# ducha-aiki/affnet

Measured on NVIDIA H100. Metric: Mpix/s end-to-end HesAffNet(+OriNet)+HardNet, higher is better.
Workload: dtype fp16 operands (fp16 residual planes: AffNet/OriNet weights+activations, HardNet layer 2-3 weights), fp32 accumulate; stencils fp32

## Files before the change

affnet_b200/csrc/pyramid.cu:

```cuda
#include <math.h>
#include <stdarg.h>

#include <string>
#include <vector>

#include <cuda.h>

#include "common.cuh"
#include "pyramid_fused.cuh"

namespace ag {

static thread_local char g_err[512] = "";
thread_local int g_launches = 0;

void set_error(const char* fmt, ...) {
    va_list ap;
    va_start(ap, fmt);
    vsnprintf(g_err, sizeof(g_err), fmt, ap);
    va_end(ap);
}

struct Prof {
    bool on = false;
    cudaStream_t st = nullptr;
    std::vector<cudaEvent_t> ev;
    std::vector<std::string> names;
    std::vector<float> ms;
};
static Prof g_prof;

void prof_mark(const char* name) {
    if (!g_prof.on) return;
    cudaEvent_t e;
    if (cudaEventCreate(&e) != cudaSuccess) return;
    cudaEventRecord(e, g_prof.st);
    g_prof.ev.push_back(e);
    g_prof.names.push_back(name);
}

constexpr int kMaxRadius = 12;
struct BlurTaps {
    int r;
    float w[2 * kMaxRadius + 1];
};

int gauss_kernel_size(double sigma) {
    int k = (int)(2.0 * 3.0 * sigma + 1.0);
    if (k % 2 == 0) k += 1;
    return k;
}

int make_taps(double sigma, BlurTaps* t) {
    int k = gauss_kernel_size(sigma);
    if (k < 1 || k > 2 * kMaxRadius + 1) {
        set_error("gaussian sigma %.4f needs %d taps (max %d)", sigma, k, 2 * kMaxRadius + 1);
        return AG_ERR_INVALID;
    }
    double half = k / 2.0, e[2 * kMaxRadius + 1], sum = 0.0;
    double step = (k > 1) ? (2.0 * half) / (k - 1) : 0.0;
    for (int i = 0; i < k; i++) {
        double x = (i == k - 1) ? half : -half + i * step;
        e[i] = exp(-(x * x) / (2.0 * sigma * sigma));
        sum += e[i];
    }
    t->r = k / 2;
    for (int i = 0; i < k; i++) t->w[i] = (float)(e[i] / sum);
    return AG_OK;
}

constexpr int TW = 64, TH = 64, NT = 256;

template <int R>
struct BlurGeom {
    static constexpr int IH = TH + 2 * R;
    static constexpr int IWQ = (TW + 2 * R + 3) / 4 + 1;
    static constexpr int IW = IWQ * 4;
    static constexpr int NQ = (4 + 2 * R + 3) / 4 + 1;
    static constexpr size_t SMEM = sizeof(float) * ((size_t)IH * IW + (size_t)IH * TW);
};

template <int R>
__global__ void __launch_bounds__(NT) blur_kernel(const float* __restrict__ in, float* __restrict__ out,
                                                   float* __restrict__ dec, int h, int w, BlurTaps taps,
                                                   const __grid_constant__ CUtensorMap tmap, int use_tmap) {
    using G = BlurGeom<R>;
    extern __shared__ __align__(128) float smem_f[];
    float* s_in = smem_f;
    float* s_mid = smem_f + G::IH * G::IW;
    constexpr int R4 = (R + 3) / 4 * 4;
    const int b = blockIdx.z;
    const int x0 = blockIdx.x * TW, y0 = blockIdx.y * TH;
    const float* img = in + (size_t)b * h * w;
#ifndef AG_BLUR_SCALAR_FILL
    const bool wide = (w & 3) == 0 && x0 - R4 >= 0 && x0 - R4 + G::IW <= w && (reinterpret_cast<size_t>(img) & 15) == 0;
#ifndef AG_BLUR_LDG_FILL
    __shared__ __align__(8) unsigned long long s_bar;
    const bool bulk = wide && y0 - R >= 0 && y0 - R + G::IH <= h;
    if (bulk) {
        const uint32_t bar = (uint32_t)__cvta_generic_to_shared(&s_bar);
        if (threadIdx.x == 0) {
            asm volatile("mbarrier.init.shared::cta.b64 [%0], 1;" ::"r"(bar));
            asm volatile("fence.mbarrier_init.release.cluster;" ::: "memory");
            asm volatile("mbarrier.arrive.expect_tx.shared::cta.b64 _, [%0], %1;" ::"r"(bar), "r"((uint32_t)(G::IH * G::IW * 4)) : "memory");
        }
        __syncthreads();
        if (use_tmap) {
            if (threadIdx.x == 0)
                asm volatile("cp.async.bulk.tensor.3d.shared::cluster.global.tile.mbarrier::complete_tx::bytes [%0], [%1, {%2, %3, %4}], [%5];" ::"r"(
                                 (uint32_t)__cvta_generic_to_shared(s_in)),
                             "l"(reinterpret_cast<uint64_t>(&tmap)), "r"(x0 - R4), "r"(y0 - R), "r"(b), "r"(bar)
                             : "memory");
        } else if ((threadIdx.x & 31) == 0) {
            const float* src = img + (size_t)(y0 - R) * w + (x0 - R4);
            for (int ly = threadIdx.x >> 5; ly < G::IH; ly += NT / 32)
                asm volatile("cp.async.bulk.shared::cluster.global.mbarrier::complete_tx::bytes [%0], [%1], %2, [%3];" ::"r"(
                                 (uint32_t)__cvta_generic_to_shared(s_in + ly * G::IW)),
                             "l"(src + (size_t)ly * w), "r"((uint32_t)(G::IW * 4)), "r"(bar)
                             : "memory");
        }
        if (threadIdx.x < 32)
            asm volatile("{\n .reg .pred P;\n W_%=:\n mbarrier.try_wait.parity.shared::cta.b64 P, [%0], 0;\n @P bra D_%=;\n bra W_%=;\n D_%=:\n}\n" ::"r"(bar) : "memory");
    } else
#endif
    if (wide) {
        constexpr int QW = G::IW / 4;
        static_assert(G::IW % 4 == 0, "window rows are whole float4s");
        for (int i = threadIdx.x; i < G::IH * QW; i += NT) {
            const int ly = i / QW, q = i - ly * QW;
            const int gy = clampi(y0 + ly - R, 0, h - 1);
            reinterpret_cast<float4*>(s_in)[i] = __ldg(reinterpret_cast<const float4*>(img + (size_t)gy * w + (x0 - R4)) + q);
        }
    } else
#endif
    for (int i = threadIdx.x; i < G::IH * G::IW; i += NT) {
        const int ly = i / G::IW, lx = i - ly * G::IW;
        const int gy = clampi(y0 + ly - R, 0, h - 1), gx = clampi(x0 + lx - R4, 0, w - 1);
        s_in[i] = __ldg(img + (size_t)gy * w + gx);
    }
    __syncthreads();
    for (int i = threadIdx.x; i < G::IH * (TW / 4); i += NT) {
        const int ly = i / (TW / 4), q = i - ly * (TW / 4);
        constexpr int OFF = R4 - R;
        float v[G::NQ * 4];
        const float4* row = reinterpret_cast<const float4*>(s_in + ly * G::IW + q * 4);
#pragma unroll
        for (int j = 0; j < G::NQ; j++) {
            const float4 t = row[j];
            v[4 * j] = t.x; v[4 * j + 1] = t.y; v[4 * j + 2] = t.z; v[4 * j + 3] = t.w;
        }
        float4 o = make_float4(0.f, 0.f, 0.f, 0.f);
#pragma unroll
        for (int k = 0; k <= 2 * R; k++) {
            const float wk = taps.w[k];
            o.x = fmaf(wk, v[OFF + k], o.x); o.y = fmaf(wk, v[OFF + k + 1], o.y);
            o.z = fmaf(wk, v[OFF + k + 2], o.z); o.w = fmaf(wk, v[OFF + k + 3], o.w);
        }
        *reinterpret_cast<float4*>(s_mid + ly * TW + q * 4) = o;
    }
    __syncthreads();
    const int h2 = (h + 1) >> 1, w2 = (w + 1) >> 1;
    const bool vec_ok = (w & 3) == 0 && (reinterpret_cast<size_t>(out) & 15) == 0;
    {
        const int q = threadIdx.x & 15, rb = threadIdx.x >> 4;
        float4 acc[4];
#pragma unroll
        for (int r = 0; r < 4; r++) acc[r] = make_float4(0.f, 0.f, 0.f, 0.f);
#pragma unroll
        for (int k = 0; k < 4 + 2 * R; k++) {
            const float4 t = *reinterpret_cast<const float4*>(s_mid + (rb * 4 + k) * TW + q * 4);
#pragma unroll
            for (int r = 0; r < 4; r++) {
                const int tap = k - r;
                if (tap >= 0 && tap <= 2 * R) {
                    const float wk = taps.w[tap];
                    acc[r].x = fmaf(wk, t.x, acc[r].x); acc[r].y = fmaf(wk, t.y, acc[r].y);
                    acc[r].z = fmaf(wk, t.z, acc[r].z); acc[r].w = fmaf(wk, t.w, acc[r].w);
                }
            }
        }
        const int gx = x0 + q * 4;
#pragma unroll
        for (int r = 0; r < 4; r++) {
            const int gy = y0 + rb * 4 + r;
            if (gy >= h || gx >= w) continue;
            float* orow = out + (size_t)b * h * w + (size_t)gy * w + gx;
            const float vals[4] = {acc[r].x, acc[r].y, acc[r].z, acc[r].w};
            if (vec_ok) {
                *reinterpret_cast<float4*>(orow) = acc[r];
            } else {
#pragma unroll
                for (int e = 0; e < 4; e++)
                    if (gx + e < w) orow[e] = vals[e];
            }
            if (dec != nullptr && (gy & 1) == 0) {
                float* drow = dec + (size_t)b * h2 * w2 + (size_t)(gy >> 1) * w2 + (gx >> 1);
                drow[0] = vals[0];
                if (gx + 2 < w) drow[1] = vals[2];
            }
        }
    }
}

typedef CUresult (*TmapEncodeFn)(CUtensorMap*, CUtensorMapDataType, cuuint32_t, void*, const cuuint64_t*, const cuuint64_t*, const cuuint32_t*,
                                 const cuuint32_t*, CUtensorMapInterleave, CUtensorMapSwizzle, CUtensorMapL2promotion, CUtensorMapFloatOOBfill);
static TmapEncodeFn tmap_encoder() {
    static TmapEncodeFn fn = nullptr;
    static bool tried = false;
    if (!tried) {
        tried = true;
        if (getenv("AG_BLUR_NO_TMA") == nullptr) {
            void* p = nullptr;
            cudaDriverEntryPointQueryResult q;
            if (cudaGetDriverEntryPoint("cuTensorMapEncodeTiled", &p, cudaEnableDefault, &q) == cudaSuccess && q == cudaDriverEntryPointSuccess)
                fn = reinterpret_cast<TmapEncodeFn>(p);
            else
                cudaGetLastError();
        }
    }
    return fn;
}

static bool make_level_tmap(CUtensorMap* m, const float* base, int B, int h, int w, int iw, int ih) {
    TmapEncodeFn enc = tmap_encoder();
    if (enc == nullptr || (w & 3) != 0 || (reinterpret_cast<size_t>(base) & 15) != 0 || iw > 256 || ih > 256) return false;
    const cuuint64_t dims[3] = {(cuuint64_t)w, (cuuint64_t)h, (cuuint64_t)B};
    const cuuint64_t strides[2] = {(cuuint64_t)w * 4, (cuuint64_t)w * h * 4};
    const cuuint32_t box[3] = {(cuuint32_t)iw, (cuuint32_t)ih, 1};
    const cuuint32_t estr[3] = {1, 1, 1};
    return enc(m, CU_TENSOR_MAP_DATA_TYPE_FLOAT32, 3, const_cast<float*>(base), dims, strides, box, estr, CU_TENSOR_MAP_INTERLEAVE_NONE,
               CU_TENSOR_MAP_SWIZZLE_NONE, CU_TENSOR_MAP_L2_PROMOTION_NONE, CU_TENSOR_MAP_FLOAT_OOB_FILL_NONE) == CUDA_SUCCESS;
}

static int launch_blur(const float* in, float* out, float* dec, int B, int h, int w, double sigma, cudaStream_t st) {
    BlurTaps taps;
    int rc = make_taps(sigma, &taps);
    if (rc != AG_OK) return rc;
    dim3 grid(cdiv(w, TW), cdiv(h, TH), B), block(NT);
    CUtensorMap tmap;
    memset(&tmap, 0, sizeof(tmap));
    switch (taps.r) {
#define AG_BLUR_CASE(R)                                                                                                   \
    case R: {                                                                                                             \
        static SmemAttrOnce attr_once;                                                                                    \
        rc = attr_once.ensure(blur_kernel<R>, BlurGeom<R>::SMEM, "blur smem attr");                                       \
        if (rc != AG_OK) return rc;                                                                                       \
        const int use_tmap = make_level_tmap(&tmap, in, B, h, w, BlurGeom<R>::IW, BlurGeom<R>::IH) ? 1 : 0;                 \
        blur_kernel<R><<<grid, block, BlurGeom<R>::SMEM, st>>>(in, out, dec, h, w, taps, tmap, use_tmap);                  \
    } break;
        AG_BLUR_CASE(1) AG_BLUR_CASE(2) AG_BLUR_CASE(3) AG_BLUR_CASE(4) AG_BLUR_CASE(5) AG_BLUR_CASE(6)
        AG_BLUR_CASE(7) AG_BLUR_CASE(8) AG_BLUR_CASE(9) AG_BLUR_CASE(10) AG_BLUR_CASE(11) AG_BLUR_CASE(12)
#undef AG_BLUR_CASE
        default:
            set_error("unsupported blur radius %d", taps.r);
            return AG_ERR_INVALID;
    }
    AG_CHECK_LAUNCH("blur_kernel");
    return AG_OK;
}

static int g_pyr_fused = 0;

static int num_sms_pyr() {
    static int n = 0;
    if (n == 0) {
        int dev = 0;
        cudaGetDevice(&dev);
        cudaDeviceGetAttribute(&n, cudaDevAttrMultiProcessorCount, dev);
        if (n <= 0) n = 148;
    }
    return n;
}

template <int CH>
static int launch_octave(const float* src, float* const* outs, float* dec, int seed, int B, int h, int w, const double* sigmas, cudaStream_t st, bool* handled) {
    using C = pf::Chain<CH>;
    *handled = false;
    if ((w & 3) != 0 || w < 8 || h < 2) return AG_OK;
    if ((reinterpret_cast<size_t>(src) & 15) || (dec && (reinterpret_cast<size_t>(dec) & 15))) return AG_OK;
    for (int l = 0; l < C::NB; l++)
        if (reinterpret_cast<size_t>(outs[l]) & 15) return AG_OK;
    pf::OctArgs a;
    memset(&a, 0, sizeof(a));
    for (int l = 0; l < C::NB; l++) {
        BlurTaps t;
        int rc = make_taps(sigmas[l], &t);
        if (rc != AG_OK) return rc;
        if (t.r != C::R(l)) return AG_OK;
        for (int k = 0; k <= 2 * t.r; k++) a.taps[l][k] = t.w[k];
        a.out[l] = outs[l];
    }
    a.src = src; a.dec = dec; a.seed = seed; a.B = B; a.h = h; a.w = w;
    a.nstrips = cdiv(w, pf::SWMAX);
    a.sw = cdiv(cdiv(w, a.nstrips), 4) * 4;
    a.nstrips = cdiv(w, a.sw);
    int nb = (2 * num_sms_pyr() + a.nstrips * B - 1) / (a.nstrips * B);
    const int nb_max = h / 48 > 1 ? h / 48 : 1;
    if (nb > nb_max) nb = nb_max;
    if (nb < 1) nb = 1;
    a.band = cdiv(h, nb);
    a.nbands = cdiv(h, a.band);
    static bool configured[64] = {};
    int dev = 0;
    cudaGetDevice(&dev);
    if (!configured[dev & 63]) {
        int rc = check_cuda(cudaFuncSetAttribute(pf::octave_kernel<CH>, cudaFuncAttributeMaxDynamicSharedMemorySize, (int)sizeof(pf::Smem<CH>)), "octave smem attr");
        if (rc != AG_OK) return rc;
        configured[dev & 63] = true;
    }
    pf::octave_kernel<CH><<<dim3(a.nstrips * a.nbands, B), 64 * C::NB, sizeof(pf::Smem<CH>), st>>>(a);
    AG_CHECK_LAUNCH("octave_kernel");
    *handled = true;
    return AG_OK;
}

__global__ void decimate_kernel(const float* __restrict__ in, float* __restrict__ out, int h, int w, int h2, int w2) {
    int x = blockIdx.x * blockDim.x + threadIdx.x, y = blockIdx.y, b = blockIdx.z;
    if (x < w2) out[(size_t)b * h2 * w2 + (size_t)y * w2 + x] = in[(size_t)b * h * w + (size_t)(2 * y) * w + 2 * x];
}

}

using namespace ag;

extern "C" {

const char* ag_last_error(void) { return ag::g_err; }
int ag_abi_version(void) { return 1; }

int ag_prof_begin(void* stream) {
    for (cudaEvent_t e : g_prof.ev) cudaEventDestroy(e);
    g_prof.ev.clear(); g_prof.names.clear(); g_prof.ms.clear();
    g_prof.st = (cudaStream_t)stream;
    g_prof.on = true;
    prof_mark("<begin>");
    return AG_OK;
}

int ag_prof_end(void) {
    g_prof.on = false;
    if (g_prof.ev.empty()) return 0;
    int rc = check_cuda(cudaEventSynchronize(g_prof.ev.back()), "prof sync");
    if (rc != AG_OK) return rc;
    g_prof.ms.assign(g_prof.ev.size(), 0.f);
    for (size_t i = 1; i < g_prof.ev.size(); i++) cudaEventElapsedTime(&g_prof.ms[i], g_prof.ev[i - 1], g_prof.ev[i]);
    return (int)g_prof.ev.size() - 1;
}

int ag_prof_get(int i, const char** name, float* ms) {
    AG_REQUIRE(i >= 0 && (size_t)(i + 1) < g_prof.ev.size() && name && ms, "index out of range");
    *name = g_prof.names[i + 1].c_str();
    *ms = g_prof.ms[i + 1];
    return AG_OK;
}

int ag_pyramid_plan(int B, int H, int W, int nlevels, double init_sigma, int border, ag_pyramid_plan_t* plan) {
    AG_REQUIRE(plan != nullptr, "plan is NULL");
    AG_REQUIRE(B >= 1 && H >= 1 && W >= 1, "bad image size");
    AG_REQUIRE(nlevels >= 1 && nlevels + 2 <= AG_MAX_LEVELS, "nlevels out of range");
    memset(plan, 0, sizeof(*plan));
    plan->B = B; plan->H = H; plan->W = W;
    plan->n_levels = nlevels + 2;
    const double sigma_step = pow(2.0, 1.0 / (double)nlevels);
    const int min_size = 2 * border + 2 + 1;
    double cur_sigma = 0.5, first = 0.0, pd = 1.0;
    if (init_sigma > cur_sigma) {
        first = sqrt(init_sigma * init_sigma - cur_sigma * cur_sigma);
        cur_sigma = init_sigma;
    }
    int h = H, w = W, o = 0;
    long long off = 0;
    for (;;) {
        AG_REQUIRE(o < AG_MAX_OCTAVES, "too many octaves");
        plan->h[o] = h; plan->w[o] = w; plan->pix_dist[o] = pd;
        plan->sigma[o][0] = cur_sigma;
        plan->blur_sigma[o][0] = (o == 0) ? first : 0.0;
        for (int l = 0; l < plan->n_levels; l++) {
            plan->level_offset[o][l] = off;
            off += (long long)B * h * w;
        }
        for (int i = 1; i < plan->n_levels; i++) {
            plan->blur_sigma[o][i] = cur_sigma * sqrt(sigma_step * sigma_step - 1.0);
            cur_sigma = cur_sigma * sigma_step;
            plan->sigma[o][i] = cur_sigma;
        }
        o++;
        pd *= 2.0;
        cur_sigma = init_sigma;
        int nh = (h + 1) / 2, nw = (w + 1) / 2;
        if (nh <= min_size || nw <= min_size) break;
        h = nh; w = nw;
    }
    plan->n_octaves = o;
    plan->total_floats = off;
    return AG_OK;
}

int ag_debug_pyramid_mode(int fused) {
    const int old = g_pyr_fused;
    g_pyr_fused = fused ? 1 : 0;
    return old;
}

int ag_gaussian_blur(const float* d_in, float* d_out, int B, int h, int w, double sigma, void* stream) {
    AG_REQUIRE(d_in && d_out && B >= 1 && h >= 1 && w >= 1, "bad arguments");
    return launch_blur(d_in, d_out, nullptr, B, h, w, sigma, (cudaStream_t)stream);
}

int ag_pyramid_build(const ag_pyramid_plan_t* p, const float* d_img, float* d_pyr, void* stream) {
    AG_REQUIRE(p && d_img && d_pyr, "NULL argument");
    cudaStream_t st = (cudaStream_t)stream;
    const int nl = p->n_levels, seed_level = nl - 2;
    for (int o = 0; o < p->n_octaves; o++)
        for (int l = (o == 0 && p->blur_sigma[0][0] > 0.0) ? 0 : 1; l < nl; l++) {
            BlurTaps t;
            int rc = make_taps(p->blur_sigma[o][l], &t);
            if (rc != AG_OK) return rc;
        }
    static const bool env_fused = getenv("AG_PYR_FUSED") != nullptr;
    const bool no_fused = !(env_fused || g_pyr_fused);
    for (int o = 0; o < p->n_octaves; o++) {
        const int h = p->h[o], w = p->w[o];
        float* lvl0 = d_pyr + p->level_offset[o][0];
        float* next0 = (o + 1 < p->n_octaves) ? d_pyr + p->level_offset[o + 1][0] : nullptr;
        if (nl == 5 && !no_fused) {
            bool handled = false;
            int rc;
            if (o == 0 && p->blur_sigma[0][0] > 0.0) {
                float* outs[5];
                double sg[5];
                for (int l = 0; l < 5; l++) { outs[l] = d_pyr + p->level_offset[0][l]; sg[l] = p->blur_sigma[0][l]; }
                rc = launch_octave<0>(d_img, outs, next0, seed_level, p->B, h, w, sg, st, &handled);
            } else if (o > 0) {
                float* outs[4];
                double sg[4];
                for (int l = 1; l < 5; l++) { outs[l - 1] = d_pyr + p->level_offset[o][l]; sg[l - 1] = p->blur_sigma[o][l]; }
                rc = launch_octave<1>(lvl0, outs, next0, seed_level - 1, p->B, h, w, sg, st, &handled);
            } else rc = AG_OK;
            if (rc != AG_OK) return rc;
            if (handled) continue;
        }
        if (o == 0) {
            if (p->blur_sigma[0][0] > 0.0) {
                int rc = launch_blur(d_img, lvl0, nullptr, p->B, h, w, p->blur_sigma[0][0], st);
                if (rc != AG_OK) return rc;
            } else {
                int rc = check_cuda(cudaMemcpyAsync(lvl0, d_img, sizeof(float) * (size_t)p->B * h * w,
                                                    cudaMemcpyDeviceToDevice, st), "copy level 0");
                if (rc != AG_OK) return rc;
            }
        }
        for (int l = 1; l < nl; l++) {
            float* dec = (l == seed_level && o + 1 < p->n_octaves) ? d_pyr + p->level_offset[o + 1][0] : nullptr;
            int rc = launch_blur(d_pyr + p->level_offset[o][l - 1], d_pyr + p->level_offset[o][l], dec, p->B, h, w,
                                 p->blur_sigma[o][l], st);
            if (rc != AG_OK) return rc;
        }
    }
    return AG_OK;
}

}
```

Baseline: 670.7.

## Fuse small-octave pyramid tail into one shared-memory kernel per image

From octave 3 onward, once the octave fits in shared memory, all remaining blur levels and decimations are built by a single per-image kernel that keeps working planes in shared memory. This removes the many small per-level blur launches whose fixed overhead dominates at small resolutions. The tail is handled with only B blocks, so it uses few SMs and could be slow if B is small. It also requires identical taps across the tail octaves and falls back to the old path otherwise.

```diff
diff --git a/affnet_b200/csrc/pyramid.cu b/affnet_b200/csrc/pyramid.cu
--- a/affnet_b200/csrc/pyramid.cu
+++ b/affnet_b200/csrc/pyramid.cu
@@ -202,6 +202,107 @@
     }
 }
 
+constexpr int TAIL_NT = 1024;
+
+struct TailArgs {
+    const float* seed;
+    float* lvl[AG_MAX_OCTAVES][AG_MAX_LEVELS];
+    int h[AG_MAX_OCTAVES], w[AG_MAX_OCTAVES];
+    int r[AG_MAX_LEVELS];
+    float taps[AG_MAX_LEVELS][2 * kMaxRadius + 1];
+    int n_oct, nl, seed_level;
+};
+
+template <int R>
+__device__ __forceinline__ void tail_hpass(const float* __restrict__ a, float* __restrict__ m, int h, int w, const float* __restrict__ wt) {
+    const int nq = (w + 3) >> 2;
+    for (int i = threadIdx.x; i < h * nq; i += TAIL_NT) {
+        const int y = i / nq, x0 = (i - y * nq) * 4;
+        const float* row = a + y * w;
+        float v[4 + 2 * R];
+#pragma unroll
+        for (int j = 0; j < 4 + 2 * R; j++) v[j] = row[clampi(x0 - R + j, 0, w - 1)];
+        float o[4] = {0.f, 0.f, 0.f, 0.f};
+#pragma unroll
+        for (int k = 0; k <= 2 * R; k++) {
+            const float wk = wt[k];
+#pragma unroll
+            for (int e = 0; e < 4; e++) o[e] = fmaf(wk, v[k + e], o[e]);
+        }
+#pragma unroll
+        for (int e = 0; e < 4; e++)
+            if (x0 + e < w) m[y * w + x0 + e] = o[e];
+    }
+}
+
+template <int R>
+__device__ __forceinline__ void tail_vpass(const float* __restrict__ m, float* __restrict__ a, float* __restrict__ g, float* __restrict__ d,
+                                           float* __restrict__ gd, int h, int w, const float* __restrict__ wt) {
+    const int nr = (h + 3) >> 2, w2 = (w + 1) >> 1;
+    for (int i = threadIdx.x; i < nr * w; i += TAIL_NT) {
+        const int yq = i / w, x = i - yq * w, y0 = yq * 4;
+        float v[4 + 2 * R];
+#pragma unroll
+        for (int j = 0; j < 4 + 2 * R; j++) v[j] = m[clampi(y0 - R + j, 0, h - 1) * w + x];
+        float o[4] = {0.f, 0.f, 0.f, 0.f};
+#pragma unroll
+        for (int k = 0; k <= 2 * R; k++) {
+            const float wk = wt[k];
+#pragma unroll
+            for (int e = 0; e < 4; e++) o[e] = fmaf(wk, v[k + e], o[e]);
+        }
+#pragma unroll
+        for (int e = 0; e < 4; e++) {
+            const int y = y0 + e;
+            if (y >= h) break;
+            a[y * w + x] = o[e];
+            g[y * w + x] = o[e];
+            if (d != nullptr && ((y | x) & 1) == 0) {
+                d[(y >> 1) * w2 + (x >> 1)] = o[e];
+                if (gd != nullptr) gd[(y >> 1) * w2 + (x >> 1)] = o[e];
+            }
+        }
+    }
+}
+
+__global__ void __launch_bounds__(TAIL_NT) pyramid_tail_kernel(const __grid_constant__ TailArgs p) {
+    extern __shared__ __align__(16) float tail_smem[];
+    const int b = blockIdx.x;
+    const int h0 = p.h[0], w0 = p.w[0];
+    float* a = tail_smem;
+    float* m = a + h0 * w0;
+    float* d = m + h0 * w0;
+    {
+        const float* src = p.seed + (size_t)b * h0 * w0;
+        for (int i = threadIdx.x; i < h0 * w0; i += TAIL_NT) a[i] = src[i];
+    }
+    for (int o = 0; o < p.n_oct; o++) {
+        const int h = p.h[o], w = p.w[o];
+        if (o > 0)
+            for (int i = threadIdx.x; i < h * w; i += TAIL_NT) a[i] = d[i];
+        __syncthreads();
+        for (int l = 1; l < p.nl; l++) {
+            const float* wt = p.taps[l];
+            float* g = p.lvl[o][l] + (size_t)b * h * w;
+            const bool seed = l == p.seed_level && o + 1 < p.n_oct;
+            float* gd = seed ? p.lvl[o + 1][0] + (size_t)b * p.h[o + 1] * p.w[o + 1] : nullptr;
+            switch (p.r[l]) {
+#define AG_TAIL_CASE(RR)                                                             \
+    case RR:                                                                         \
+        tail_hpass<RR>(a, m, h, w, wt);                                              \
+        __syncthreads();                                                             \
+        tail_vpass<RR>(m, a, g, seed ? d : nullptr, gd, h, w, wt);                   \
+        break;
+                AG_TAIL_CASE(1) AG_TAIL_CASE(2) AG_TAIL_CASE(3) AG_TAIL_CASE(4) AG_TAIL_CASE(5) AG_TAIL_CASE(6)
+                AG_TAIL_CASE(7) AG_TAIL_CASE(8) AG_TAIL_CASE(9) AG_TAIL_CASE(10) AG_TAIL_CASE(11) AG_TAIL_CASE(12)
+#undef AG_TAIL_CASE
+                default: break;
+            }
+            __syncthreads();
+        }
+    }
+}
+
 typedef CUresult (*TmapEncodeFn)(CUtensorMap*, CUtensorMapDataType, cuuint32_t, void*, const cuuint64_t*, const cuuint64_t*, const cuuint32_t*,
                                  const cuuint32_t*, CUtensorMapInterleave, CUtensorMapSwizzle, CUtensorMapL2promotion, CUtensorMapFloatOOBfill);
 static TmapEncodeFn tmap_encoder() {
@@ -259,6 +360,54 @@
     return AG_OK;
 }
 
+constexpr int kTailFirstOctave = 3, kTailMaxPixels = 4 * TW * TH;
+
+static int launch_tail(const ag_pyramid_plan_t* p, int first, float* d_pyr, cudaStream_t st, bool* handled) {
+    *handled = false;
+    const int nl = p->n_levels, n = p->n_octaves - first;
+    if (first < kTailFirstOctave || n < 1) return AG_OK;
+    const int h0 = p->h[first], w0 = p->w[first];
+    if (h0 * w0 > kTailMaxPixels) return AG_OK;
+    const size_t smem = sizeof(float) * (2 * (size_t)h0 * w0 + (size_t)((h0 + 1) / 2) * ((w0 + 1) / 2));
+    static int optin = 0;
+    if (optin == 0) {
+        int dev = 0;
+        cudaGetDevice(&dev);
+        cudaDeviceGetAttribute(&optin, cudaDevAttrMaxSharedMemoryPerBlockOptin, dev);
+        if (optin <= 0) optin = 48 * 1024;
+    }
+    if (smem > (size_t)optin) return AG_OK;
+    TailArgs a;
+    memset(&a, 0, sizeof(a));
+    for (int l = 1; l < nl; l++) {
+        BlurTaps t;
+        int rc = make_taps(p->blur_sigma[first][l], &t);
+        if (rc != AG_OK) return rc;
+        a.r[l] = t.r;
+        for (int k = 0; k <= 2 * t.r; k++) a.taps[l][k] = t.w[k];
+        for (int o = first + 1; o < p->n_octaves; o++) {
+            BlurTaps u;
+            rc = make_taps(p->blur_sigma[o][l], &u);
+            if (rc != AG_OK) return rc;
+            if (u.r != t.r || memcmp(u.w, t.w, sizeof(float) * (2 * t.r + 1)) != 0) return AG_OK;
+        }
+    }
+    a.seed = d_pyr + p->level_offset[first][0];
+    for (int o = 0; o < n; o++) {
+        a.h[o] = p->h[first + o];
+        a.w[o] = p->w[first + o];
+        for (int l = 0; l < nl; l++) a.lvl[o][l] = d_pyr + p->level_offset[first + o][l];
+    }
+    a.n_oct = n; a.nl = nl; a.seed_level = nl - 2;
+    static SmemAttrOnce attr_once;
+    int rc = attr_once.ensure(pyramid_tail_kernel, smem, "tail smem attr");
+    if (rc != AG_OK) return rc;
+    pyramid_tail_kernel<<<p->B, TAIL_NT, smem, st>>>(a);
+    AG_CHECK_LAUNCH("pyramid_tail_kernel");
+    *handled = true;
+    return AG_OK;
+}
+
 static int g_pyr_fused = 0;
 
 static int num_sms_pyr() {
@@ -420,6 +569,10 @@
     static const bool env_fused = getenv("AG_PYR_FUSED") != nullptr;
     const bool no_fused = !(env_fused || g_pyr_fused);
     for (int o = 0; o < p->n_octaves; o++) {
+        bool tail = false;
+        int rc = launch_tail(p, o, d_pyr, st, &tail);
+        if (rc != AG_OK) return rc;
+        if (tail) break;
         const int h = p->h[o], w = p->w[o];
         float* lvl0 = d_pyr + p->level_offset[o][0];
         float* next0 = (o + 1 < p->n_octaves) ? d_pyr + p->level_offset[o + 1][0] : nullptr;
```

Result: no change. 669.8, median of 6 (-0.1%).
